# bcollico/Deep-Multiview-Depth-Estimation

Measured on AMD Instinct MI355X. Metric: depth maps/sec + warp-kernel HBM GB/s, 3-view 640x512 D=192, 1/2/4/8 GPU, higher is better.
Workload: dtype f32

## Files before the change

deep-multiview-depth-estimation_amd/csrc/conv3d_region.hip:

```cpp
#include <cstdlib>

#include "launchers.h"
#include "region_conv.h"

namespace mvs {
namespace {

struct Geo {
  int n[3];
  int o0[3];
  int on[3];
  int i0[3];
  int in[3];
  int pad[3];
  int out_cf;
  int in_c4;
  const uint32_t* absmax;
  uint32_t* y_bound;
  int st0[3];
  int stn[3];
};

__device__ inline void store_out(float* __restrict__ y, const Geo& g, int b, int co, int vz, int vy, int vx,
                                 int CO, float v) {
  const size_t vox = ((size_t)(vz + g.st0[0]) * g.stn[1] + (vy + g.st0[1])) * g.stn[2] + (vx + g.st0[2]);
  const size_t rvol = (size_t)g.stn[0] * g.stn[1] * g.stn[2];
  if (g.out_cf) y[((size_t)b * CO + co) * rvol + vox] = v;
  else y[((size_t)b * rvol + vox) * CO + co] = v;
}

template <int MODE, int CI, int CO, int RB, int QM, int CLS, int PS = 1>
__device__ __forceinline__ void region_conv(
    const float* __restrict__ x, const float* __restrict__ x2, const float* __restrict__ w,
    float* __restrict__ y, const float* __restrict__ bn_scale, const float* __restrict__ bn_shift,
    const float* __restrict__ bn_mean, const Geo& g) {
  constexpr int NB = CO / 16;
  static_assert(CI % 16 == 0 && CO % 16 == 0, "channel counts in multiples of 16");
  static_assert((MODE == kT2) == (CLS >= 0), "parity classes: transposed convolutions");
  static_assert(PS == 1 || (PS == 4 && CI == 112) || (PS == 3 && MODE == kS2 && QM == 4),
                "partial sums: the input gradients only");
  static_assert(QM != 4 || MODE == kS2, "channels-last volume: the stride-2 mode");
  constexpr bool kPlanes = MODE == kS2 && QM != 4;
  const int lane = (int)threadIdx.x & 63;
  const int m = lane & 15, kq = lane >> 4;
  const int b = (int)blockIdx.z;

  int cf[3], cn[3];
  constexpr int par[3] = {CLS >= 0 ? (CLS >> 2) & 1 : 0, CLS >= 0 ? (CLS >> 1) & 1 : 0, CLS >= 0 ? CLS & 1 : 0};
  if constexpr (MODE == kT2) {
#pragma unroll
    for (int d = 0; d < 3; ++d) class_dim(g.o0[d], g.on[d], g.pad[d], par[d], cf[d], cn[d]);
  } else {
#pragma unroll
    for (int d = 0; d < 3; ++d) {
      cf[d] = g.o0[d];
      cn[d] = g.on[d];
    }
  }
  const int rows = cn[0] * cn[1] * cn[2];
  const int sx = QM == 3 ? cv_split_exponent(g.absmax) : 0;
  const int step = MODE == kT2 ? 2 : 1;
  constexpr int kRows = 16 * RB;
  const int bx = xcd_work_id((int)blockIdx.x, (int)gridDim.x);
  const int row0 = (bx * (kBlock / 64) + ((int)threadIdx.x >> 6)) * kRows;
  if (row0 >= rows) return;

  int lim[3];
#pragma unroll
  for (int d = 0; d < 3; ++d) lim[d] = g.in[d];
  int lin[RB];
  unsigned vm[RB][3];
#pragma unroll
  for (int rb = 0; rb < RB; ++rb) {
    const int r = row0 + rb * 16 + m;
    const bool ok = r < rows;
    const int rr = ok ? r : 0;
    const int jx = rr % cn[2], t = rr / cn[2];
    const int jy = t % cn[1], jz = t / cn[1];
    const int o[3] = {cf[0] + step * jz, cf[1] + step * jy, cf[2] + step * jx};
    int bs[3];
#pragma unroll
    for (int d = 0; d < 3; ++d) {
      if constexpr (MODE == kS1) bs[d] = o[d] - 1 - g.i0[d];
      else if constexpr (MODE == kS2) bs[d] = 2 * o[d] - g.pad[d] - g.i0[d];
      else bs[d] = ((o[d] + g.pad[d] - par[d]) >> 1) - g.i0[d];
      unsigned mk = 0;
#pragma unroll
      for (int tt = 0; tt < 3; ++tt) {
        const int dl = MODE == kT2 ? -(tt >> 1) : tt;
        const bool in = ok && bs[d] + dl >= 0 && bs[d] + dl < lim[d] && !(MODE == kT2 && ((tt & 1) != par[d]));
        mk |= in ? (1u << tt) : 0u;
      }
      vm[rb][d] = mk;
    }
    lin[rb] = (bs[0] * lim[1] + bs[1]) * lim[2] + bs[2];
  }

  f4v acc[PS][RB][NB];
#pragma unroll
  for (int ps = 0; ps < PS; ++ps)
#pragma unroll
    for (int rb = 0; rb < RB; ++rb)
#pragma unroll
      for (int nb = 0; nb < NB; ++nb) acc[ps][rb][nb] = f4v{0.0f, 0.0f, 0.0f, 0.0f};

  const size_t rvol = (size_t)g.in[0] * g.in[1] * g.in[2];
  const int sy = lim[2], sz = lim[1] * lim[2];
#pragma unroll
  for (int tz = 0; tz < 3; ++tz) {
    if (MODE == kT2 && ((tz & 1) != par[0])) continue;
#pragma unroll
    for (int ty = 0; ty < 3; ++ty) {
      if (MODE == kT2 && ((ty & 1) != par[1])) continue;
      const int dz = MODE == kT2 ? -(tz >> 1) : tz, dy = MODE == kT2 ? -(ty >> 1) : ty;
      uint32_t vox[3][RB];
#pragma unroll
      for (int tx = 0; tx < 3; ++tx)
#pragma unroll
        for (int rb = 0; rb < RB; ++rb) {
          const int dx = MODE == kT2 ? -(tx >> 1) : tx;
          const bool ok = ((vm[rb][0] >> tz) & (vm[rb][1] >> ty) & (vm[rb][2] >> tx) & 1u) != 0;
          vox[tx][rb] = ok ? (uint32_t)(lin[rb] + dz * sz + dy * sy + dx) : kOob;
        }
#pragma unroll
      for (int cb = 0; cb < CI / 16; ++cb) {
        const int c4 = cb * 16 + kq * 4;
        const int ps = PS == 1 ? 0 : PS == 3 ? tz : (cb + 1) / 2;
        Rsrc rs, rs2;
        if constexpr (kPlanes) {
          if constexpr (QM == 2)
            rs = make_rsrc(reinterpret_cast<const char*>(x) + ((size_t)b * (CI / 4) + cb * 4) * rvol * 8,
                           (uint32_t)(rvol * 32));
          else if constexpr (QM == 1 || QM == 3)
            rs = make_rsrc(x + ((size_t)b * (CI / 4) + cb * 4) * rvol * 4, (uint32_t)(rvol * 64));
          else
            rs = make_rsrc(x + ((size_t)b * CI + cb * 16) * rvol, (uint32_t)(rvol * 64));
        } else {
          rs = make_rsrc(x + (size_t)b * rvol * CI, (uint32_t)(rvol * CI * 4));
          if (x2) rs2 = make_rsrc(x2 + (size_t)b * rvol * CI, (uint32_t)(rvol * CI * 4));
        }
        f4v a[3][RB], bw[3][NB];
#pragma unroll
        for (int tx = 0; tx < 3; ++tx) {
          if (MODE == kT2 && ((tx & 1) != par[2])) continue;
#pragma unroll
          for (int rb = 0; rb < RB; ++rb) {
            const uint32_t vx = vox[tx][rb];
            f4v v;
            if constexpr (kPlanes) {
              if constexpr (QM == 2) {
                typedef __attribute__((ext_vector_type(2))) unsigned v2u;
                const v2u p = __builtin_amdgcn_raw_buffer_load_b64(
                    rs, (int)(vx == kOob ? kOob : ((uint32_t)kq * (uint32_t)rvol + vx) * 8u), 0, 0);
                v = f4v{__uint_as_float(p.x << 16), __uint_as_float(p.x & 0xFFFF0000u),
                          __uint_as_float(p.y << 16), __uint_as_float(p.y & 0xFFFF0000u)};
              } else if constexpr (QM == 3) {
                v = unsplit4(__builtin_bit_cast(uint4, __builtin_amdgcn_raw_buffer_load_b128(
                                 rs, (int)(vx == kOob ? kOob : ((uint32_t)kq * (uint32_t)rvol + vx) * 16u), 0, 0)),
                             sx);
              } else if constexpr (QM == 1) {
                v = ld4(rs, vx == kOob ? kOob : ((uint32_t)kq * (uint32_t)rvol + vx) * 16u, 0);
              } else {
#pragma unroll
                for (int q = 0; q < 4; ++q)
                  v[q] = __uint_as_float(__builtin_amdgcn_raw_buffer_load_b32(
                      rs, (int)(vx == kOob ? kOob : ((uint32_t)(kq * 4 + q) * (uint32_t)rvol + vx) * 4u), 0, 0));
              }
            } else {
              const uint32_t eo = vx == kOob ? kOob : (vx * (uint32_t)CI + (uint32_t)c4) * 4u;
              v = ld4(rs, eo, 0);
              if (x2) v += ld4(rs2, eo, 0);
            }
            a[tx][rb] = v;
          }
          const float* wt = w + (size_t)((tz * 3 + ty) * 3 + tx) * CO * CI;
#pragma unroll
          for (int nb = 0; nb < NB; ++nb)
            bw[tx][nb] = *reinterpret_cast<const f4v*>(wt + (size_t)(nb * 16 + m) * CI + c4);
        }
#pragma unroll
        for (int tx = 0; tx < 3; ++tx) {
          if (MODE == kT2 && ((tx & 1) != par[2])) continue;
#pragma unroll
          for (int s = 0; s < 4; ++s)
#pragma unroll
            for (int rb = 0; rb < RB; ++rb)
#pragma unroll
              for (int nb = 0; nb < NB; ++nb)
                acc[ps][rb][nb] =
                    __builtin_amdgcn_mfma_f32_16x16x4f32(a[tx][rb][s], bw[tx][nb][s], acc[ps][rb][nb], 0, 0, 0);
        }
      }
    }
  }

  float vmax = 0.0f;
#pragma unroll
  for (int nb = 0; nb < NB; ++nb) {
    const int co = nb * 16 + m;
    const float sc = bn_scale ? bn_scale[co] : 1.0f, sh = bn_scale ? bn_shift[co] : 0.0f,
                mu = bn_scale ? bn_mean[co] : 0.0f;
#pragma unroll
    for (int rb = 0; rb < RB; ++rb)
#pragma unroll
      for (int r = 0; r < 4; ++r) {
        const int row = row0 + rb * 16 + kq * 4 + r;
        if (row >= rows) continue;
        const int jx = row % cn[2], t = row / cn[2];
        const int jy = t % cn[1], jz = t / cn[1];
        const int vz = cf[0] + step * jz - g.o0[0], vy = cf[1] + step * jy - g.o0[1],
                  vx = cf[2] + step * jx - g.o0[2];
        float v = acc[0][rb][nb][r];
        if constexpr (PS == 4)
          v = (v + acc[1][rb][nb][r]) + (acc[PS - 2][rb][nb][r] + acc[PS - 1][rb][nb][r]);
        if constexpr (PS == 3) v = (v + acc[1][rb][nb][r]) + acc[PS - 1][rb][nb][r];
        if (bn_scale) v = fmaxf((v - mu) * sc + sh, 0.0f);
        vmax = fmaxf(vmax, fabsf(v));
        store_out(y, g, b, co, vz, vy, vx, CO, v);
      }
  }
  if (g.y_bound) bound_update(g.y_bound, vmax);
}

template <int MODE, int CI, int CO, int RB, int QM = 0, int PS = 1>
__global__ __launch_bounds__(kBlock) void conv3d_region_kernel(
    const float* __restrict__ x, const float* __restrict__ x2, const float* __restrict__ w,
    float* __restrict__ y, const float* __restrict__ bn_scale, const float* __restrict__ bn_shift,
    const float* __restrict__ bn_mean, Geo g) {
  if constexpr (MODE == kT2) {
    switch (blockIdx.y) {
#define MVS_T2_CLASS(c) \
  case c: region_conv<MODE, CI, CO, RB, QM, c, PS>(x, x2, w, y, bn_scale, bn_shift, bn_mean, g); break;
      MVS_T2_CLASS(0) MVS_T2_CLASS(1) MVS_T2_CLASS(2) MVS_T2_CLASS(3)
      MVS_T2_CLASS(4) MVS_T2_CLASS(5) MVS_T2_CLASS(6) MVS_T2_CLASS(7)
#undef MVS_T2_CLASS
      default: break;
    }
  } else {
    region_conv<MODE, CI, CO, RB, QM, -1, PS>(x, x2, w, y, bn_scale, bn_shift, bn_mean, g);
  }
}

template <int MODE, int CI, int CO, int RB, int QM = 0, int PS = 1>
void launch_mode(const float* x, const float* x2, const float* w, float* y, const float* sc, const float* sh,
                 const float* mu, int B, const Geo& g, hipStream_t s) {
  hipLaunchKernelGGL((conv3d_region_kernel<MODE, CI, CO, RB, QM, PS>), region_grid(MODE, RB, B, g.on), dim3(kBlock), 0, s,
                     x, x2, w, y, sc, sh, mu, g);
}

template <int CI>
struct S1TileF {
  static constexpr int TZ = CI == 16 ? 8 : (CI == 32 ? 4 : 2);
  static constexpr int PX = 18, PY = 6, PZ = TZ + 2, PV = PX * PY * PZ;
  static constexpr int NCH = CI / 4;
  static constexpr int REC = CI * 4;
  static constexpr int LDS = PV * REC;
};

template <int CI>
__device__ inline int s1f_off(int v, int c) {
  constexpr int NCH = CI / 4;
  return v * (CI * 4) + ((c ^ (((v * NCH) >> 3) % NCH)) << 4);
}

template <int CI, int CO>
__global__ __launch_bounds__(kBlock) void conv3d_s1_lds_kernel(
    const float* __restrict__ x, const float* __restrict__ w, float* __restrict__ y,
    const float* __restrict__ bn_scale, const float* __restrict__ bn_shift, const float* __restrict__ bn_mean, Geo g,
    int tiles_x, int tiles_y, int tiles_z) {
  using T = S1TileF<CI>;
  constexpr int NB = CO / 16;
  constexpr int RB = 8;
  static_assert(T::TZ * NB == RB && CI == CO, "tile shapes");
  __shared__ __attribute__((aligned(16))) char lds[T::LDS];

  int t = xcd_work_id((int)blockIdx.x, (int)gridDim.x);
  if (t >= tiles_x * tiles_y * tiles_z) return;
  const int tx0 = (t % tiles_x) * 16;
  t /= tiles_x;
  const int ty0 = (t % tiles_y) * 4;
  t /= tiles_y;
  const int tz0 = t * T::TZ;
  const int b = (int)blockIdx.y;
  const int tid = (int)threadIdx.x, lane = tid & 63, wave = tid >> 6;
  const int m = lane & 15, kq = lane >> 4;

  {
    constexpr int NIT = T::PV * T::NCH, PER = (NIT + kBlock - 1) / kBlock, BATCH = 8;
    const size_t rvol = (size_t)g.in[0] * g.in[1] * g.in[2];
    const Rsrc rs = make_rsrc(x + (size_t)b * rvol * CI, (uint32_t)(rvol * CI * 4));
#pragma unroll
    for (int k0 = 0; k0 < PER; k0 += BATCH) {
      f4v v4[BATCH];
#pragma unroll
      for (int k = 0; k < BATCH; ++k) {
        const int e = tid + kBlock * (k0 + k);
        const int q = e % T::NCH, v = e / T::NCH;
        const int px = v % T::PX, py = (v / T::PX) % T::PY, pz = v / (T::PX * T::PY);
        const int rx = g.o0[2] + tx0 - 1 + px - g.i0[2], ry = g.o0[1] + ty0 - 1 + py - g.i0[1],
                  rz = g.o0[0] + tz0 - 1 + pz - g.i0[0];
        const bool ok = k0 + k < PER && e < NIT && rx >= 0 && rx < g.in[2] && ry >= 0 && ry < g.in[1] && rz >= 0 &&
                        rz < g.in[0];
        v4[k] = ld4(rs, ok ? (uint32_t)((((size_t)rz * g.in[1] + ry) * g.in[2] + rx) * CI + 4 * q) * 4u : kOob, 0);
      }
      __builtin_amdgcn_sched_barrier(0);
      asm volatile("s_waitcnt vmcnt(0)" ::: "memory");
      __builtin_amdgcn_sched_barrier(0);
#pragma unroll
      for (int k = 0; k < BATCH; ++k) {
        const int e = tid + kBlock * (k0 + k);
        if (k0 + k >= PER || e >= NIT) continue;
        *reinterpret_cast<f4v*>(lds + s1f_off<CI>(e / T::NCH, e % T::NCH)) = v4[k];
      }
      __builtin_amdgcn_sched_barrier(0);
      asm volatile("s_waitcnt lgkmcnt(0)" ::: "memory");
      __builtin_amdgcn_sched_barrier(0);
    }
  }
  __syncthreads();

  const int nb = wave % NB, rg = wave / NB;
  f4v acc[RB];
#pragma unroll
  for (int r = 0; r < RB; ++r) acc[r] = f4v{0.0f, 0.0f, 0.0f, 0.0f};
  const float* wn = w + (size_t)(nb * 16 + m) * CI + 4 * kq;
  f4v a[3][RB];
  auto lda = [&](int tr, int tx, int cb, f4v (&dst)[RB]) {
    const int tz = tr / 3, ty = tr % 3;
#pragma unroll
    for (int r = 0; r < RB; ++r) {
      const int rbi = rg * RB + r, zz = rbi >> 2, yy = rbi & 3;
      const int v = ((zz + tz) * T::PY + (yy + ty)) * T::PX + (m + tx);
      dst[r] = *reinterpret_cast<const f4v*>(lds + s1f_off<CI>(v, cb * 4 + kq));
    }
  };
  auto ldw = [&](int tr, int cb, f4v (&bw)[3]) {
#pragma unroll
    for (int tx = 0; tx < 3; ++tx)
      bw[tx] = *reinterpret_cast<const f4v*>(wn + (size_t)((tr * 3 + tx) * CO) * CI + cb * 16);
  };
  constexpr int CB = CI / 16, NIT = 9 * CB;
  f4v bw[3], bn_[3];
  ldw(0, 0, bw);
  lda(0, 0, 0, a[0]);
#pragma unroll 1
  for (int it = 0; it < NIT; ++it) {
    const int tr = it / CB, cb = it % CB;
    const bool more = it + 1 < NIT;
    const int tr1 = (it + 1) / CB, cb1 = (it + 1) % CB;
    if (more) ldw(tr1, cb1, bn_);
#pragma unroll
    for (int tx = 0; tx < 3; ++tx) {
      if (tx < 2) lda(tr, tx + 1, cb, a[tx + 1]);
      else if (more) lda(tr1, 0, cb1, a[0]);
#pragma unroll
      for (int s = 0; s < 4; ++s)
#pragma unroll
        for (int r = 0; r < RB; ++r)
          acc[r] = __builtin_amdgcn_mfma_f32_16x16x4f32(a[tx][r][s], bw[tx][s], acc[r], 0, 0, 0);
    }
#pragma unroll
    for (int tx = 0; tx < 3; ++tx) bw[tx] = bn_[tx];
  }

  const int co = nb * 16 + m;
  const float sc = bn_scale ? bn_scale[co] : 1.0f, sh = bn_scale ? bn_shift[co] : 0.0f,
              mu = bn_scale ? bn_mean[co] : 0.0f;
  float vmax = 0.0f;
#pragma unroll
  for (int r = 0; r < RB; ++r) {
    const int rbi = rg * RB + r, zz = rbi >> 2, yy = rbi & 3;
    if (tz0 + zz >= g.on[0] || ty0 + yy >= g.on[1]) continue;
#pragma unroll
    for (int i = 0; i < 4; ++i) {
      if (tx0 + 4 * kq + i >= g.on[2]) continue;
      float v = acc[r][i];
      if (bn_scale) v = fmaxf((v - mu) * sc + sh, 0.0f);
      vmax = fmaxf(vmax, fabsf(v));
      store_out(y, g, b, co, tz0 + zz, ty0 + yy, tx0 + 4 * kq + i, CO, v);
    }
  }
  if (g.y_bound) bound_update(g.y_bound, vmax);
}

template <int CI>
void launch_s1_lds(const float* x, const float* w, float* y, const float* sc, const float* sh, const float* mu,
                   int B, const Geo& g, hipStream_t s) {
  const int tx = (g.on[2] + 15) / 16, ty = (g.on[1] + 3) / 4, tz = (g.on[0] + S1TileF<CI>::TZ - 1) / S1TileF<CI>::TZ;
  hipLaunchKernelGGL((conv3d_s1_lds_kernel<CI, CI>), tile_grid(tx * ty * tz, B), dim3(kBlock), 0, s, x, w, y, sc, sh,
                     mu, g, tx, ty, tz);
}

}

int launch_conv3d_region(int mode, bool out_cf, int in_c4, const float* x, const float* x2, const float* w,
                         float* y, int B, int CI, int CO, const int* n, const int* o0, const int* on, const int* i0,
                         const int* in, const int* pad, const float* bn_scale, const float* bn_shift,
                         const float* bn_mean, hipStream_t s, const uint32_t* absmax, uint32_t* y_bound,
                         bool per_lane, const int* st0, const int* stn, bool s2_lds) {
  Geo g;
  g.y_bound = y_bound;
  g.out_cf = out_cf ? 1 : 0;
  g.in_c4 = in_c4;
  g.absmax = absmax;
  for (int d = 0; d < 3; ++d) {
    g.n[d] = n[d];
    g.o0[d] = o0[d];
    g.on[d] = on[d];
    g.i0[d] = i0 ? i0[d] : 0;
    g.in[d] = in ? in[d] : n[d];
    g.pad[d] = pad ? pad[d] : 1;
    g.st0[d] = st0 ? st0[d] : 0;
    g.stn[d] = stn ? stn[d] : on[d];
  }
  static const bool s1_lds = [] {
    const char* e = getenv("MVS_FP32_S1_LDS");
    return e && e[0] == '1';
  }();
  if (mode == kS1 && !x2 && CI == CO && !per_lane && s1_lds) {
    if (CI == 16) return launch_s1_lds<16>(x, w, y, bn_scale, bn_shift, bn_mean, B, g, s), MVS_OK;
    if (CI == 32) return launch_s1_lds<32>(x, w, y, bn_scale, bn_shift, bn_mean, B, g, s), MVS_OK;
    if (CI == 64) return launch_s1_lds<64>(x, w, y, bn_scale, bn_shift, bn_mean, B, g, s), MVS_OK;
  }
  if (mode == kS2 && CI == 32 && CO == 16 && (in_c4 == 0 || in_c4 == 1) && !x2 && !absmax && !y_bound &&
      !per_lane && !st0 && !stn && !i0 && !in && !out_cf && pad && (s2_lds || conv_s2_lds_enabled()) &&
      (uint64_t)n[0] * (uint64_t)n[1] * (uint64_t)n[2] * 128u < 0xFFFFFFF0ull) {
    launch_conv_s2_lds(x, in_c4, w, y, B, n, o0, on, pad, bn_scale, bn_shift, bn_mean, s);
    return MVS_OK;
  }
  static const int s2_rb = [] {
    const char* e = getenv("MVS_S2_RB");
    return e && e[0] == '4' ? 4 : 2;
  }();
  if (mode == kS2 && in_c4 == 1 && CI == 32 && s2_rb == 4) {
    if (CO == 16) return launch_mode<kS2, 32, 16, 4, 1>(x, x2, w, y, bn_scale, bn_shift, bn_mean, B, g, s), MVS_OK;
    if (CO == 32) return launch_mode<kS2, 32, 32, 4, 1>(x, x2, w, y, bn_scale, bn_shift, bn_mean, B, g, s), MVS_OK;
  }
#define MVS_REGION_CASE(MD, A, C)                                                       \
  if (mode == MD && CI == A && CO == C) {                                               \
    launch_mode<MD, A, C, 2>(x, x2, w, y, bn_scale, bn_shift, bn_mean, B, g, s);        \
    return MVS_OK;                                                                      \
  }
#define MVS_REGION_S2(A, C)                                                                                   \
  if (mode == kS2 && CI == A && CO == C) {                                                                    \
    if (in_c4 == 3) launch_mode<kS2, A, C, 2, 3>(x, x2, w, y, bn_scale, bn_shift, bn_mean, B, g, s);         \
    else if (in_c4 == 2) launch_mode<kS2, A, C, 2, 2>(x, x2, w, y, bn_scale, bn_shift, bn_mean, B, g, s);    \
    else if (in_c4) launch_mode<kS2, A, C, 2, 1>(x, x2, w, y, bn_scale, bn_shift, bn_mean, B, g, s);         \
    else launch_mode<kS2, A, C, 2, 0>(x, x2, w, y, bn_scale, bn_shift, bn_mean, B, g, s);                    \
    return MVS_OK;                                                                                            \
  }
  MVS_REGION_S2(32, 16) MVS_REGION_S2(32, 32) MVS_REGION_S2(32, 64)
  MVS_REGION_CASE(kS1, 16, 16) MVS_REGION_CASE(kS1, 32, 32) MVS_REGION_CASE(kS1, 64, 64)
  static const int t2_rb = [] {
    const char* e = getenv("MVS_T2_RB");
    return e && e[0] == '4' ? 4 : e && e[0] == '2' ? 2 : 0;
  }();
  if (mode == kT2 && CI == 64 && CO == 32 && t2_rb == 4)
    return launch_mode<kT2, 64, 32, 4>(x, x2, w, y, bn_scale, bn_shift, bn_mean, B, g, s), MVS_OK;
  if (mode == kT2 && CI == 32 && CO == 16 && t2_rb != 2)
    return launch_mode<kT2, 32, 16, 4>(x, x2, w, y, bn_scale, bn_shift, bn_mean, B, g, s), MVS_OK;
  MVS_REGION_CASE(kT2, 64, 32) MVS_REGION_CASE(kT2, 32, 16)
#undef MVS_REGION_CASE
#undef MVS_REGION_S2
  return MVS_ERR_INVALID_ARGUMENT;
}

void launch_conv3d_s2_dgrad(const float* gy, const float* w27, float* gx, int B, const int* n, const int* pad_lo,
                            const int* out, hipStream_t s) {
  Geo g;
  g.y_bound = nullptr;
  g.absmax = nullptr;
  g.out_cf = 1;
  g.in_c4 = 0;
  for (int d = 0; d < 3; ++d) {
    g.n[d] = n[d];
    g.o0[d] = 0;
    g.on[d] = n[d];
    g.i0[d] = 0;
    g.in[d] = out[d];
    g.pad[d] = pad_lo[d];
    g.st0[d] = 0;
    g.stn[d] = n[d];
  }
  launch_mode<kT2, 112, 32, 2, 0, 4>(gy, nullptr, w27, gx, nullptr, nullptr, nullptr, B, g, s);
}

int launch_conv3d_t2_dgrad(const float* gy, const float* w27, float* gx, int B, int CC, int CF, const int* in,
                           const int* crop, const int* out, hipStream_t s) {
  Geo g;
  g.y_bound = nullptr;
  g.absmax = nullptr;
  g.out_cf = 0;
  g.in_c4 = 0;
  for (int d = 0; d < 3; ++d) {
    g.n[d] = out[d];
    g.o0[d] = 0;
    g.on[d] = in[d];
    g.i0[d] = 0;
    g.in[d] = out[d];
    g.pad[d] = crop[d];
    g.st0[d] = 0;
    g.stn[d] = in[d];
  }
  if (CC == 64 && CF == 32) launch_mode<kS2, 32, 64, 2, 4, 3>(gy, nullptr, w27, gx, nullptr, nullptr, nullptr, B, g, s);
  else if (CC == 32 && CF == 16)
    launch_mode<kS2, 16, 32, 2, 4, 3>(gy, nullptr, w27, gx, nullptr, nullptr, nullptr, B, g, s);
  else return MVS_ERR_INVALID_ARGUMENT;
  return MVS_OK;
}

}
```

deep-multiview-depth-estimation_amd/csrc/region_conv.h:

```cpp
#pragma once
#include "common.h"
#include "packed.h"
#include "split.h"

namespace mvs {

typedef _Float16 h8v __attribute__((ext_vector_type(8)));
constexpr uint32_t kOob = 0xFFFFFFC0u;
constexpr int kS1 = 0, kS2 = 1, kT2 = 2;

__device__ __forceinline__ void class_dim(int o0, int on, int p, int par, int& first, int& cnt) {
  first = o0 + (((o0 + p) & 1) != par ? 1 : 0);
  cnt = first < o0 + on ? (o0 + on - 1 - first) / 2 + 1 : 0;
}

inline dim3 region_grid(int mode, int RB, int B, const int* on) {
  const bool t2 = mode == kT2;
  const long rows = (long)(t2 ? (on[0] + 1) / 2 : on[0]) * (t2 ? (on[1] + 1) / 2 : on[1]) *
                    (t2 ? (on[2] + 1) / 2 : on[2]);
  const long per_block = (kBlock / 64) * 16 * RB;
  return dim3(xcd_grid((int)((rows + per_block - 1) / per_block)).x, t2 ? 8u : 1u, (unsigned)B);
}

inline dim3 tile_grid(int tiles, int B) { return dim3(xcd_grid(tiles).x, (unsigned)B); }

template <int CI>
struct SplitRec {
  static constexpr int REC = CI * 4;
  static constexpr int NCH = REC / 16;
  __device__ __forceinline__ static int chunk_off(int v, int c) {
    return v * REC + ((c ^ ((v / (16 / NCH)) % NCH)) << 4);
  }
};

__device__ __forceinline__ void mfma3(const h8v& ahi, const h8v& alo, const h8v& bhi, const h8v& blo, f4v& acc) {
  acc = __builtin_amdgcn_mfma_f32_16x16x32_f16(ahi, bhi, acc, 0, 0, 0);
  acc = __builtin_amdgcn_mfma_f32_16x16x32_f16(ahi, blo, acc, 0, 0, 0);
  acc = __builtin_amdgcn_mfma_f32_16x16x32_f16(alo, bhi, acc, 0, 0, 0);
}

__device__ __forceinline__ h8v wfrag(const h8v* __restrict__ wf, int kb, int NB, int nb, int part, int lane) {
  return wf[((size_t)(kb * NB + nb) * 2 + part) * 64 + lane];
}

}
```

Before: 684.1.

## Add cell-based transposed-conv kernel computing all eight parity classes per wave

```diff
diff --git a/deep-multiview-depth-estimation_amd/csrc/conv3d_region.hip b/deep-multiview-depth-estimation_amd/csrc/conv3d_region.hip
--- a/deep-multiview-depth-estimation_amd/csrc/conv3d_region.hip
+++ b/deep-multiview-depth-estimation_amd/csrc/conv3d_region.hip
@@ -246,6 +246,189 @@
                  const float* mu, int B, const Geo& g, hipStream_t s) {
   hipLaunchKernelGGL((conv3d_region_kernel<MODE, CI, CO, RB, QM, PS>), region_grid(MODE, RB, B, g.on), dim3(kBlock), 0, s,
                      x, x2, w, y, sc, sh, mu, g);
+}
+
+typedef float f2v __attribute__((ext_vector_type(2)));
+
+template <int A>
+__device__ __forceinline__ void store_run8(float* __restrict__ p, const float (&v)[8], int lo, int hi) {
+  auto st1 = [&](int i) {
+    if (i >= lo && i < hi) p[i] = v[i];
+  };
+  auto st2 = [&](int i) {
+    if (i >= lo && i + 2 <= hi) *reinterpret_cast<f2v*>(p + i) = f2v{v[i], v[i + 1]};
+    else st1(i), st1(i + 1);
+  };
+  auto st4 = [&](int i) {
+    if (i >= lo && i + 4 <= hi) *reinterpret_cast<f4v*>(p + i) = f4v{v[i], v[i + 1], v[i + 2], v[i + 3]};
+    else st2(i), st2(i + 2);
+  };
+  if constexpr (A == 0) st4(0), st4(4);
+  else if constexpr (A == 2) st2(0), st4(2), st2(6);
+  else if constexpr (A == 1) st1(0), st2(1), st4(3), st1(7);
+  else st1(0), st4(1), st2(5), st1(7);
+}
+
+template <int CI, int CO, int RB, bool X2>
+__global__ __launch_bounds__(kBlock) void conv3d_t2_cells_kernel(
+    const float* __restrict__ x, const float* __restrict__ x2, const float* __restrict__ w,
+    float* __restrict__ y, const float* __restrict__ bn_scale, const float* __restrict__ bn_shift,
+    const float* __restrict__ bn_mean, Geo g) {
+  constexpr int NB = CO / 16, CB = CI / 16;
+  static_assert(CI % 16 == 0 && CO % 16 == 0, "channel counts in multiples of 16");
+  const int lane = (int)threadIdx.x & 63;
+  const int m = lane & 15, kq = lane >> 4;
+  const int b = (int)blockIdx.z;
+
+  int cf[3], cn[3];
+#pragma unroll
+  for (int d = 0; d < 3; ++d) cell_dim(g.o0[d], g.on[d], g.pad[d], cf[d], cn[d]);
+  const int nbx = (cn[2] + 15) >> 4;
+  const int blocks = cn[0] * cn[1] * nbx;
+  const int bx = xcd_work_id((int)blockIdx.x, (int)gridDim.x);
+  const int blk0 = uniform((bx * (kBlock / 64) + ((int)threadIdx.x >> 6)) * RB);
+  if (blk0 >= blocks) return;
+
+  const int sy = g.in[2], sz = g.in[1] * g.in[2];
+  bool live[RB];
+  int lz[RB], ly[RB], xb[RB], lin[RB];
+  unsigned vm[RB][3];
+#pragma unroll
+  for (int rb = 0; rb < RB; ++rb) {
+    live[rb] = blk0 + rb < blocks;
+    const int blk = live[rb] ? blk0 + rb : 0;
+    xb[rb] = blk % nbx;
+    const int line = blk / nbx;
+    ly[rb] = line % cn[1];
+    lz[rb] = line / cn[1];
+    const int ci[3] = {lz[rb], ly[rb], xb[rb] * 16 + m};
+    int bs[3];
+#pragma unroll
+    for (int d = 0; d < 3; ++d) {
+      bs[d] = cf[d] + ci[d] - g.i0[d];
+      unsigned mk = 0;
+#pragma unroll
+      for (int j = 0; j < 2; ++j)
+        mk |= (live[rb] && ci[d] < cn[d] && bs[d] - j >= 0 && bs[d] - j < g.in[d]) ? (1u << j) : 0u;
+      vm[rb][d] = mk;
+    }
+    lin[rb] = (bs[0] * g.in[1] + bs[1]) * g.in[2] + bs[2];
+  }
+
+  f4v acc[8][RB][NB];
+#pragma unroll
+  for (int c = 0; c < 8; ++c)
+#pragma unroll
+    for (int rb = 0; rb < RB; ++rb)
+#pragma unroll
+      for (int nb = 0; nb < NB; ++nb) acc[c][rb][nb] = f4v{0.0f, 0.0f, 0.0f, 0.0f};
+
+  const size_t rvol_in = (size_t)g.in[0] * g.in[1] * g.in[2];
+  const Rsrc rs = make_rsrc(x + (size_t)b * rvol_in * CI, (uint32_t)(rvol_in * CI * 4));
+  Rsrc rs2;
+  if constexpr (X2) rs2 = make_rsrc(x2 + (size_t)b * rvol_in * CI, (uint32_t)(rvol_in * CI * 4));
+
+  constexpr int kRowOrder[9][2] = {{0, 0}, {0, 1}, {1, 0}, {1, 1}, {0, 2}, {1, 2}, {2, 0}, {2, 1}, {2, 2}};
+  f4v a[RB][2][CB];
+#pragma unroll
+  for (int it = 0; it < 9; ++it) {
+    const int tz = kRowOrder[it][0], ty = kRowOrder[it][1];
+    const int jz = tz >> 1, jy = ty >> 1;
+    if (it == 0 || it == 4 || it == 6 || it == 8) {
+#pragma unroll
+      for (int rb = 0; rb < RB; ++rb)
+#pragma unroll
+        for (int jx = 0; jx < 2; ++jx) {
+          const bool ok = ((vm[rb][0] >> jz) & (vm[rb][1] >> jy) & (vm[rb][2] >> jx) & 1u) != 0;
+          const uint32_t vo = (uint32_t)(lin[rb] - jz * sz - jy * sy - jx) * (uint32_t)(CI * 4) + (uint32_t)kq * 16u;
+#pragma unroll
+          for (int cb = 0; cb < CB; ++cb) {
+            const uint32_t eo = ok ? vo + (uint32_t)cb * 64u : kOob;
+            f4v v = ld4(rs, eo, 0);
+            if constexpr (X2) v += ld4(rs2, eo, 0);
+            a[rb][jx][cb] = v;
+          }
+        }
+    }
+#pragma unroll
+    for (int cb = 0; cb < CB; ++cb) {
+      const int c4 = cb * 16 + kq * 4;
+      f4v bw[3][NB];
+#pragma unroll
+      for (int tx = 0; tx < 3; ++tx) {
+        const float* wt = w + (size_t)((tz * 3 + ty) * 3 + tx) * CO * CI;
+#pragma unroll
+        for (int nb = 0; nb < NB; ++nb)
+          bw[tx][nb] = *reinterpret_cast<const f4v*>(wt + (size_t)(nb * 16 + m) * CI + c4);
+      }
+#pragma unroll
+      for (int tx = 0; tx < 3; ++tx) {
+        const int cls = ((tz & 1) << 2) | ((ty & 1) << 1) | (tx & 1);
+#pragma unroll
+        for (int s = 0; s < 4; ++s)
+#pragma unroll
+          for (int rb = 0; rb < RB; ++rb)
+#pragma unroll
+            for (int nb = 0; nb < NB; ++nb)
+              acc[cls][rb][nb] = __builtin_amdgcn_mfma_f32_16x16x4f32(a[rb][tx >> 1][cb][s], bw[tx][nb][s],
+                                                                      acc[cls][rb][nb], 0, 0, 0);
+      }
+    }
+  }
+
+  const size_t rvol = (size_t)g.stn[0] * g.stn[1] * g.stn[2];
+#pragma unroll
+  for (int rb = 0; rb < RB; ++rb) {
+    const int vx0 = 2 * (cf[2] + xb[rb] * 16 + kq * 4) - g.pad[2] - g.o0[2];
+    const int lo = vx0 < 0 ? -vx0 : 0, hi = g.on[2] - vx0 < 8 ? g.on[2] - vx0 : 8;
+#pragma unroll
+    for (int nb = 0; nb < NB; ++nb) {
+      const int co = nb * 16 + m;
+      const float sc = bn_scale ? bn_scale[co] : 1.0f, sh = bn_scale ? bn_shift[co] : 0.0f,
+                  mu = bn_scale ? bn_mean[co] : 0.0f;
+#pragma unroll
+      for (int pzy = 0; pzy < 4; ++pzy) {
+        const int vz = 2 * (cf[0] + lz[rb]) + (pzy >> 1) - g.pad[0] - g.o0[0];
+        const int vy = 2 * (cf[1] + ly[rb]) + (pzy & 1) - g.pad[1] - g.o0[1];
+        if (!live[rb] || vz < 0 || vz >= g.on[0] || vy < 0 || vy >= g.on[1] || lo >= hi) continue;
+        float v[8];
+#pragma unroll
+        for (int i = 0; i < 8; ++i) {
+          float t = acc[pzy * 2 + (i & 1)][rb][nb][i >> 1];
+          if (bn_scale) t = fmaxf((t - mu) * sc + sh, 0.0f);
+          v[i] = t;
+        }
+        const long vox = ((long)(vz + g.st0[0]) * g.stn[1] + (vy + g.st0[1])) * g.stn[2] + (vx0 + g.st0[2]);
+        if (g.out_cf) {
+          const long e = (long)(((size_t)b * CO + co) * rvol) + vox;
+          float* p = y + e;
+          switch ((int)((reinterpret_cast<uintptr_t>(p) >> 2) & 3)) {
+            case 0: store_run8<0>(p, v, lo, hi); break;
+            case 1: store_run8<1>(p, v, lo, hi); break;
+            case 2: store_run8<2>(p, v, lo, hi); break;
+            default: store_run8<3>(p, v, lo, hi); break;
+          }
+        } else {
+          float* p = y + ((long)((size_t)b * rvol) + vox) * CO + co;
+#pragma unroll
+          for (int i = 0; i < 8; ++i)
+            if (i >= lo && i < hi) p[(long)i * CO] = v[i];
+        }
+      }
+    }
+  }
+}
+
+constexpr int kCellsRB = 2;
+
+template <int CI, int CO, int RB>
+void launch_t2_cells(const float* x, const float* x2, const float* w, float* y, const float* sc, const float* sh,
+                     const float* mu, int B, const Geo& g, hipStream_t s) {
+  const dim3 grid = cell_grid(RB, B, g.o0, g.on, g.pad);
+  if (x2)
+    hipLaunchKernelGGL((conv3d_t2_cells_kernel<CI, CO, RB, true>), grid, dim3(kBlock), 0, s, x, x2, w, y, sc, sh, mu, g);
+  else
+    hipLaunchKernelGGL((conv3d_t2_cells_kernel<CI, CO, RB, false>), grid, dim3(kBlock), 0, s, x, x2, w, y, sc, sh, mu, g);
 }
 
 template <int CI>
@@ -451,15 +634,11 @@
   }
   MVS_REGION_S2(32, 16) MVS_REGION_S2(32, 32) MVS_REGION_S2(32, 64)
   MVS_REGION_CASE(kS1, 16, 16) MVS_REGION_CASE(kS1, 32, 32) MVS_REGION_CASE(kS1, 64, 64)
-  static const int t2_rb = [] {
-    const char* e = getenv("MVS_T2_RB");
-    return e && e[0] == '4' ? 4 : e && e[0] == '2' ? 2 : 0;
-  }();
-  if (mode == kT2 && CI == 64 && CO == 32 && t2_rb == 4)
-    return launch_mode<kT2, 64, 32, 4>(x, x2, w, y, bn_scale, bn_shift, bn_mean, B, g, s), MVS_OK;
-  if (mode == kT2 && CI == 32 && CO == 16 && t2_rb != 2)
+  if (mode == kT2 && CI == 32 && CO == 16 && !per_lane && !y_bound && on[0] > 0 && on[1] > 0 && on[2] > 0)
+    return launch_t2_cells<32, 16, kCellsRB>(x, x2, w, y, bn_scale, bn_shift, bn_mean, B, g, s), MVS_OK;
+  if (mode == kT2 && CI == 32 && CO == 16)
     return launch_mode<kT2, 32, 16, 4>(x, x2, w, y, bn_scale, bn_shift, bn_mean, B, g, s), MVS_OK;
-  MVS_REGION_CASE(kT2, 64, 32) MVS_REGION_CASE(kT2, 32, 16)
+  MVS_REGION_CASE(kT2, 64, 32)
 #undef MVS_REGION_CASE
 #undef MVS_REGION_S2
   return MVS_ERR_INVALID_ARGUMENT;
diff --git a/deep-multiview-depth-estimation_amd/csrc/region_conv.h b/deep-multiview-depth-estimation_amd/csrc/region_conv.h
--- a/deep-multiview-depth-estimation_amd/csrc/region_conv.h
+++ b/deep-multiview-depth-estimation_amd/csrc/region_conv.h
@@ -14,12 +14,25 @@
   cnt = first < o0 + on ? (o0 + on - 1 - first) / 2 + 1 : 0;
 }
 
+__host__ __device__ __forceinline__ void cell_dim(int o0, int on, int p, int& first, int& cnt) {
+  first = (o0 + p) >> 1;
+  cnt = ((o0 + on - 1 + p) >> 1) - first + 1;
+}
+
 inline dim3 region_grid(int mode, int RB, int B, const int* on) {
   const bool t2 = mode == kT2;
   const long rows = (long)(t2 ? (on[0] + 1) / 2 : on[0]) * (t2 ? (on[1] + 1) / 2 : on[1]) *
                     (t2 ? (on[2] + 1) / 2 : on[2]);
   const long per_block = (kBlock / 64) * 16 * RB;
   return dim3(xcd_grid((int)((rows + per_block - 1) / per_block)).x, t2 ? 8u : 1u, (unsigned)B);
+}
+
+inline dim3 cell_grid(int RB, int B, const int* o0, const int* on, const int* pad) {
+  int cf[3], cn[3];
+  for (int d = 0; d < 3; ++d) cell_dim(o0[d], on[d], pad[d], cf[d], cn[d]);
+  const long blocks = (long)cn[0] * cn[1] * ((cn[2] + 15) / 16);
+  const long waves = (blocks + RB - 1) / RB, per_block = kBlock / 64;
+  return dim3(xcd_grid((int)((waves + per_block - 1) / per_block)).x, 1u, (unsigned)B);
 }
 
 inline dim3 tile_grid(int tiles, int B) { return dim3(xcd_grid(tiles).x, (unsigned)B); }
```

New measurement: 702.2, median of 6. +2.6%, better.
